# RemcoHoger/Space-Filling-Curves-for-Vision-Transformers

Measured on AMD Instinct MI355X. Metric: images/sec ViT-B/16 224px Hilbert-order training, higher is better.
Workload: dtype bf16; 1 GPU; vit_b16_224_hilbert: 224x224 Hilbert pixel order, 16x16-pixel tokens, batch 256/GPU, full train step (fwd+CE+bwd+clip+AdamW); global_batch=256, parallelism=dp1, hip_graph=False

## Files before the change

### space-filling-curves-for-vision-transformers_amd/csrc/gemm8p.hip

```cpp
#include "common_host.h"
#include "gemm_core.h"
#include <mutex>
#include <type_traits>
#include <unordered_map>

namespace sfcvit {
namespace {

using namespace gemm_core;

namespace p8 {

constexpr int T = 512, HALF = 16384, KTB = 65536, LDS_BYTES = 2 * KTB;
constexpr int LDS_TQ = LDS_BYTES, LDS_PATCH = LDS_TQ + 64, LDS_BIAS = LDS_PATCH + 8 * 2048, LDS_MAX = P8_LDS_MAX;
static_assert(LDS_BIAS == P8_LDS_BIAS, "dispatch.h prices the bias vector at this offset");
enum { RELU = P8_RELU, DROP = P8_DROP, RES = P8_RES, DACT = P8_DACT, CSUM = P8_CSUM, BITS = P8_BITS };

typedef const __attribute__((address_space(1))) void *gptr_t;
typedef __attribute__((address_space(3))) void *lptr_t;

template <int N> __device__ __forceinline__ void wait_vm() { asm volatile("s_waitcnt vmcnt(%0)" ::"n"(N) : "memory"); }
template <int N> __device__ __forceinline__ void wait_lgkm() {
    asm volatile("s_waitcnt lgkmcnt(%0)" ::"n"(N) : "memory");
    __builtin_amdgcn_sched_barrier(0);
// ... 16 lines not shown
};

template <int MASK>
__device__ __forceinline__ void epilogue_math(const sfcvit_gemm_args &g, int m, int n, float (&v)[16], const float (&bv)[16],
                                              const u32x4 (&side)[2], uint32_t thresh, float keep_scale, float dact_scale,
                                              uint32_t rk_in0, uint32_t rk_in1, u32x4 &w0, u32x4 &w1) {
    if (!(MASK & DACT)) {
#pragma unroll
        for (int r = 0; r < 16; r++) v[r] += bv[r];
    }
    if (MASK & RELU) {
#pragma unroll
        for (int r = 0; r < 16; r++) v[r] = fmaxf(v[r], 0.f);
    }
    if (MASK & DROP) {
        const uint64_t row = uint64_t(m) + uint64_t(uint32_t(g.row_offset));
        const uint32_t rk = mix32(uint32_t(row) * 0x9E3779B1u + ((row >> 32) ? rk_in1 : rk_in0));
#pragma unroll
        for (int p = 0; p < 8; p++) {
            bool k0, k1;
            drop_keep2(rk, uint32_t(n >> 1) + p, thresh, k0, k1);
            v[2 * p] = k0 ? v[2 * p] * keep_scale : 0.f;
            v[2 * p + 1] = k1 ? v[2 * p + 1] * keep_scale : 0.f;
        }
    }
    if (MASK & RES) {
        float rv[16];
        unpack8f(side[0], rv);
        unpack8f(side[1], rv + 8);
#pragma unroll
        for (int r = 0; r < 16; r++) v[r] += rv[r];
    }
    if ((MASK & BITS) && (MASK & RELU)) {
        uint32_t bits = 0;
#pragma unroll
        for (int r = 0; r < 16; r++) bits |= uint32_t(v[r] > 0.f) << r;
        uint8_t *mp = static_cast<uint8_t *>(g.actmask) + size_t(m) * g.ld_actmask + (n >> 3);
        asm volatile("global_store_short %0, %1, off\n\ts_nop 1" ::"v"(mp), "v"(bits) : "memory");
    }
    if (MASK & DACT) {
        if (MASK & BITS) {
            const uint32_t bits = side[0][0];
#pragma unroll
            for (int r = 0; r < 16; r++) v[r] = (bits >> r & 1u) ? v[r] * dact_scale : 0.f;
        } else {
            float a[16];
            unpack8f(side[0], a);
            unpack8f(side[1], a + 8);
#pragma unroll
            for (int r = 0; r < 16; r++) v[r] = a[r] > 0.f ? v[r] * dact_scale : 0.f;
        }
    }
    w0 = u32x4{pack2bf(v[0], v[1]), pack2bf(v[2], v[3]), pack2bf(v[4], v[5]), pack2bf(v[6], v[7])};
    w1 = u32x4{pack2bf(v[8], v[9]), pack2bf(v[10], v[11]), pack2bf(v[12], v[13]), pack2bf(v[14], v[15])};
}

#define SFCVIT_XROW(a, b) "ds_write_b128 %[wa], " a "\n\tds_write_b128 %[wb], " b "\n\tds_read_b128 " a ", %[ra]\n\tds_read_b128 " b ", %[ra] offset:1024\n\t"
template <int NR>
__device__ __forceinline__ void patch_exchange(u32x4 (&w)[NR][2], const StoreMap &sm) {
    static_assert(NR >= 1 && NR <= 8, "rows per batch");
    const int wa = sm.wa, wb = sm.wa ^ 16, ra = sm.ra;
    if constexpr (NR == 8)
        asm volatile(SFCVIT_XROW("%0", "%1") SFCVIT_XROW("%2", "%3") SFCVIT_XROW("%4", "%5") SFCVIT_XROW("%6", "%7")
                     SFCVIT_XROW("%8", "%9") SFCVIT_XROW("%10", "%11") SFCVIT_XROW("%12", "%13") SFCVIT_XROW("%14", "%15") "s_waitcnt lgkmcnt(0)"
                     : "+v"(w[0][0]), "+v"(w[0][1]), "+v"(w[1][0]), "+v"(w[1][1]), "+v"(w[2][0]), "+v"(w[2][1]), "+v"(w[3][0]), "+v"(w[3][1]),
                       "+v"(w[4][0]), "+v"(w[4][1]), "+v"(w[5][0]), "+v"(w[5][1]), "+v"(w[6][0]), "+v"(w[6][1]), "+v"(w[7][0]), "+v"(w[7][1])
                     : [wa] "v"(wa), [wb] "v"(wb), [ra] "v"(ra) : "memory");
    else if constexpr (NR == 7)
        asm volatile(SFCVIT_XROW("%0", "%1") SFCVIT_XROW("%2", "%3") SFCVIT_XROW("%4", "%5") SFCVIT_XROW("%6", "%7")
                     SFCVIT_XROW("%8", "%9") SFCVIT_XROW("%10", "%11") SFCVIT_XROW("%12", "%13") "s_waitcnt lgkmcnt(0)"
                     : "+v"(w[0][0]), "+v"(w[0][1]), "+v"(w[1][0]), "+v"(w[1][1]), "+v"(w[2][0]), "+v"(w[2][1]), "+v"(w[3][0]), "+v"(w[3][1]),
                       "+v"(w[4][0]), "+v"(w[4][1]), "+v"(w[5][0]), "+v"(w[5][1]), "+v"(w[6][0]), "+v"(w[6][1])
                     : [wa] "v"(wa), [wb] "v"(wb), [ra] "v"(ra) : "memory");
    else if constexpr (NR == 6)
        asm volatile(SFCVIT_XROW("%0", "%1") SFCVIT_XROW("%2", "%3") SFCVIT_XROW("%4", "%5") SFCVIT_XROW("%6", "%7")
                     SFCVIT_XROW("%8", "%9") SFCVIT_XROW("%10", "%11") "s_waitcnt lgkmcnt(0)"
                     : "+v"(w[0][0]), "+v"(w[0][1]), "+v"(w[1][0]), "+v"(w[1][1]), "+v"(w[2][0]), "+v"(w[2][1]), "+v"(w[3][0]), "+v"(w[3][1]),
                       "+v"(w[4][0]), "+v"(w[4][1]), "+v"(w[5][0]), "+v"(w[5][1])
                     : [wa] "v"(wa), [wb] "v"(wb), [ra] "v"(ra) : "memory");
    else if constexpr (NR == 4)
        asm volatile(SFCVIT_XROW("%0", "%1") SFCVIT_XROW("%2", "%3") SFCVIT_XROW("%4", "%5") SFCVIT_XROW("%6", "%7") "s_waitcnt lgkmcnt(0)"
                     : "+v"(w[0][0]), "+v"(w[0][1]), "+v"(w[1][0]), "+v"(w[1][1]), "+v"(w[2][0]), "+v"(w[2][1]), "+v"(w[3][0]), "+v"(w[3][1])
                     : [wa] "v"(wa), [wb] "v"(wb), [ra] "v"(ra) : "memory");
    else
        static_assert(NR == 8, "patch_exchange: batch sizes 4, 6, 7, 8");
}
#undef SFCVIT_XROW

__device__ __forceinline__ void store_row_pair(const sfcvit_gemm_args &g, int m, int n, const StoreMap &sm, const u32x4 &w0, const u32x4 &w1) {
    uint16_t *c = static_cast<uint16_t *>(g.c) + size_t(m) * g.ldc + n + sm.coff;
    asm volatile("global_store_dwordx4 %0, %1, off sc0 sc1 nt\n\ts_nop 1" ::"v"(c), "v"(w0) : "memory");
    asm volatile("global_store_dwordx4 %0, %1, off sc0 sc1 nt\n\ts_nop 1" ::"v"(c + size_t(8) * g.ldc), "v"(w1) : "memory");
}


template <int NI, int MASK, bool P2 = false>
__global__ __launch_bounds__(T) void gemm8p_kernel(const sfcvit_gemm_args g, unsigned *__restrict__ counters, int stag_slots, int stag_ticks, int walk) {
    constexpr int BM = 32 * NI, GR = 16 * NI;
    extern __shared__ __attribute__((aligned(16))) char smem[];
    if (stag_ticks > 0) {
        const uint64_t until = __builtin_amdgcn_s_memrealtime() + uint64_t((blockIdx.x >> 3) % stag_slots) * uint64_t(stag_ticks);
        while (__builtin_amdgcn_s_memrealtime() < until) __builtin_amdgcn_s_sleep(8);
    }
    const int tid = threadIdx.x, lane = tid & 63, wid = __builtin_amdgcn_readfirstlane(tid >> 6), wr = wid >> 2, wc = wid & 3;
    const int q = lane >> 4, nl = lane & 15;
    const int K = g.K, NT = g.N / 256, ntiles = ((g.M + BM - 1) / BM) * NT, KT = K / 64, m_last = g.M - BM;
    const uint16_t *A = static_cast<const uint16_t *>(g.a);
    const uint16_t *B = static_cast<const uint16_t *>(g.b);
    const int G = gridDim.x, per_xcd = G >> 3, xcd = blockIdx.x & 7;
    int *const tq = reinterpret_cast<int *>(smem + LDS_TQ);
    auto tile_of = [&](unsigned l) __attribute__((always_inline)) {
        const long t = long(l / unsigned(per_xcd)) * G + xcd * per_xcd + int(l % unsigned(per_xcd));
        if (t >= ntiles) return -1;
        if (walk > 0 && walk < NT) {
            const unsigned MT = unsigned(ntiles / NT), full = unsigned(NT / walk) * MT * unsigned(walk), ut = unsigned(t);
            const unsigned wcur = ut < full ? unsigned(walk) : unsigned(NT % walk), base = ut < full ? (ut / (MT * walk)) * walk : unsigned(NT / walk) * walk;
            const unsigned tt = ut < full ? ut % (MT * walk) : ut - full;
            return int((tt / wcur) << 16 | (base + tt % wcur));
        }
        return int((unsigned(t) / unsigned(NT)) << 16 | (unsigned(t) % unsigned(NT)));
    };
    auto finish = [&]() __attribute__((always_inline)) {
        if (tid == 0) {
            const unsigned old = atomicAdd(counters + 8, 1u);
            if (old == unsigned(G) - 1u) {
#pragma unroll
                for (int i = 0; i < 9; i++) counters[i] = 0u;
            }
        }
    };
    if (tid == 0) {
        const unsigned l0 = atomicAdd(counters + xcd, 1u);
        tq[0] = tile_of(l0);
        const unsigned l1 = atomicAdd(counters + xcd, 1u);
        tq[1] = tile_of(l1);
    }
    const bool has_bias = !(MASK & DACT) && g.bias != nullptr;
    if (has_bias)
        for (int i = tid; i < g.N / 8; i += T)
            *reinterpret_cast<u32x4 *>(smem + LDS_BIAS + i * 16) = static_cast<const u32x4 *>(g.bias)[i];
    __syncthreads();

    int tile_cur = __builtin_amdgcn_readfirstlane(tq[0]);
    if (tile_cur < 0) { finish(); return; }
    unsigned drawn = 0;
    if (tid == 0) drawn = atomicAdd(counters + xcd, 1u);
    const int tile_first = tile_cur;
    int t = 0;

    const int r1 = 8 * wid + (lane >> 3);
    const int sc = (lane & 7) ^ ((r1 >> 1) & 7);
    const int w1 = (r1 < GR - 64) ? r1 : r1 - (NI == 7 ? 16 : 32);
    const int b_row = (r1 >> 5) * 64 + ((r1 & 15) >> 2) * 16 + ((r1 >> 4) & 1) * 4 + (r1 & 3);
    const uint32_t voffA0 = (uint32_t(r1) * uint32_t(g.lda) + sc * 8) * 2, voffA1 = (uint32_t(64 + w1) * uint32_t(g.lda) + sc * 8) * 2;
    const uint32_t voffB = (uint32_t(b_row) * uint32_t(g.ldb) + sc * 8) * 2;
    const size_t a_second = size_t(GR) * g.lda, b_second = size_t(128) * g.ldb, b_h1 = size_t(8) * g.ldb;

    auto cursor_at = [&](int seq, int tile, bool is_a) __attribute__((always_inline)) {
        Cursor c;
        c.tile = seq;
        c.k0 = 0;
        if (tile < 0) tile = tile_first;
        c.p = is_a ? A + size_t(min((tile >> 16) * BM, m_last)) * g.lda : B + size_t(tile & 0xFFFF) * 256 * g.ldb;
        return c;
    };
    const uint16_t *next_a = nullptr, *next_b = nullptr;
    auto set_next = [&](int seq) __attribute__((always_inline)) {
        const Cursor na = cursor_at(seq, __builtin_amdgcn_readfirstlane(tq[seq & 3]), true);
        const Cursor nb = cursor_at(seq, __builtin_amdgcn_readfirstlane(tq[seq & 3]), false);
        next_a = na.p;
        next_b = nb.p;
    };
    auto advance = [&](Cursor &c, bool is_a) __attribute__((always_inline)) {
        if (c.k0 + 64 == K) { c.tile++; c.k0 = 0; c.p = is_a ? next_a : next_b; }
        else { c.k0 += 64; c.p += 64; }
    };
    const int m0_wave = wid * 1024;
    auto dma16 = [&](const uint16_t *base, uint32_t voff, int lds) __attribute__((always_inline)) {
        asm volatile("s_mov_b32 m0, %2\n\ts_nop 0\n\tglobal_load_lds_dwordx4 %0, %1"
                     :
                     : "v"(voff), "s"(base), "s"(lds)
                     : "memory");
    };
    auto stage_a = [&](const Cursor &c, int buf, int h) __attribute__((always_inline)) {
        const int d = m0_wave + buf * KTB + h * HALF;
        const uint32_t vo = h ? voffA1 : voffA0;
        dma16(c.p, vo, d);
        dma16(c.p + a_second, vo, d + 8192);
    };
    auto stage_b = [&](const Cursor &c, int buf, int h) __attribute__((always_inline)) {
        const uint16_t *p = c.p + (h ? b_h1 : 0);
        const int d = m0_wave + buf * KTB + 2 * HALF + h * HALF;
        dma16(p, voffB, d);
        dma16(p + b_second, voffB, d + 8192);
    };

    const int o0 = nl * 128 + ((q ^ ((nl >> 1) & 7)) << 4);
    const int a_off0 = wr * 8192 + o0, a_off1 = wr * 8192 + (o0 ^ 64);
    const int b_off0 = 2 * HALF + wc * 4096 + o0, b_off1 = 2 * HALF + wc * 4096 + (o0 ^ 64);
    bf16x8 fa0[4][2], fa1[NI - 4][2], fb0[2][2], fb1[2][2];
    auto read_a0 = [&](int buf) __attribute__((always_inline)) {
#pragma unroll
        for (int i = 0; i < 4; i++) {
            fa0[i][0] = *reinterpret_cast<const bf16x8 *>(smem + a_off0 + buf * KTB + i * 2048);
            fa0[i][1] = *reinterpret_cast<const bf16x8 *>(smem + a_off1 + buf * KTB + i * 2048);
        }
    };
    auto read_a1 = [&](int buf) __attribute__((always_inline)) {
#pragma unroll
        for (int i = 0; i < NI - 4; i++) {
            fa1[i][0] = *reinterpret_cast<const bf16x8 *>(smem + a_off0 + buf * KTB + HALF + i * 2048);
            fa1[i][1] = *reinterpret_cast<const bf16x8 *>(smem + a_off1 + buf * KTB + HALF + i * 2048);
        }
    };
    auto read_b = [&](bf16x8 (&fb)[2][2], int buf, int sub) __attribute__((always_inline)) {
#pragma unroll
        for (int j = 0; j < 2; j++) {
            fb[j][0] = *reinterpret_cast<const bf16x8 *>(smem + b_off0 + buf * KTB + sub * HALF + j * 2048);
            fb[j][1] = *reinterpret_cast<const bf16x8 *>(smem + b_off1 + buf * KTB + sub * HALF + j * 2048);
        }
    };

    f32x4 acc[NI][4];
    auto zero_acc = [&]() __attribute__((always_inline)) {
#pragma unroll
        for (int i = 0; i < NI; i++)
#pragma unroll
            for (int j = 0; j < 4; j++) acc[i][j] = f32x4{0.f, 0.f, 0.f, 0.f};
    };
    auto mma0 = [&](const bf16x8 (&fb)[2][2], int bsub) __attribute__((always_inline)) {
        __builtin_amdgcn_s_setprio(1);
#pragma unroll
        for (int kk = 0; kk < 2; kk++)
#pragma unroll
            for (int i = 0; i < 4; i++)
#pragma unroll
                for (int j = 0; j < 2; j++)
                    acc[i][bsub * 2 + j] = __builtin_amdgcn_mfma_f32_16x16x32_bf16(fb[j][kk], fa0[i][kk], acc[i][bsub * 2 + j], 0, 0, 0);
        __builtin_amdgcn_s_setprio(0);
    };
    auto mma1 = [&](const bf16x8 (&fb)[2][2], int bsub) __attribute__((always_inline)) {
        __builtin_amdgcn_s_setprio(1);
#pragma unroll
        for (int kk = 0; kk < 2; kk++)
#pragma unroll
            for (int i = 0; i < NI - 4; i++)
#pragma unroll
                for (int j = 0; j < 2; j++)
                    acc[4 + i][bsub * 2 + j] = __builtin_amdgcn_mfma_f32_16x16x32_bf16(fb[j][kk], fa1[i][kk], acc[4 + i][bsub * 2 + j], 0, 0, 0);
        __builtin_amdgcn_s_setprio(0);
    };

    const uint32_t thresh = (MASK & DROP) ? drop_thresh(g.dropout_p) : 0u;
    const float keep_scale = (MASK & DROP) ? 1.f / (1.f - g.dropout_p) : 1.f;
    const uint32_t seed_e = (MASK & DROP) ? eff_seed(g.dropout_seed, g.seed_off) : 0u;
    const uint32_t rk_in0 = (MASK & DROP) ? mix32(seed_e) : 0u, rk_in1 = (MASK & DROP) ? mix32(seed_e ^ 0x7FEB352Du) : 0u;
    const float dact_scale = g.dact_scale != 0.f ? g.dact_scale : 1.f;
    auto draw = [&]() __attribute__((always_inline)) {
        if (tid == 0) {
            tq[(t + 2) & 3] = tile_of(drawn);
            drawn = atomicAdd(counters + xcd, 1u);
        }
    };
    auto epilogue = [&]() __attribute__((always_inline)) {
        const int tile = tile_cur;
        int te = tid;
        asm volatile("" : "+v"(te));
        const int le = te & 63, qe = le >> 4, ne = le & 15;
        StoreMap sm;
        {
            const int patch = LDS_PATCH + wid * 2048, r0 = le >> 3, ch = le & 7;
            sm.wa = patch + ne * 128 + (((2 * qe) ^ (ne & 7)) << 4);
            sm.ra = patch + r0 * 128 + ((ch ^ r0) << 4);
            sm.coff = long(r0 - ne) * g.ldc + (8 * ch - 16 * qe);
        }
        const int m_new = (tile >> 16) * BM;
        const int m0 = min(m_new, m_last) + wr * GR + ne, n0 = (tile & 0xFFFF) * 256 + wc * 64 + qe * 16;
        mfma_fence();
        float bv[16];
        if (has_bias) {
            const char *bp = smem + LDS_BIAS + n0 * 2;
            unpack8f(*reinterpret_cast<const u32x4 *>(bp), bv);
            unpack8f(*reinterpret_cast<const u32x4 *>(bp + 16), bv + 8);
        } else {
#pragma unroll
            for (int r = 0; r < 16; r++) bv[r] = 0.f;
        }
        const uint16_t *sp = (MASK & RES) ? static_cast<const uint16_t *>(g.residual) : static_cast<const uint16_t *>(g.aux_in);
        const size_t ld_side = (MASK & RES) ? size_t(g.ldr) : size_t(g.ldaux);
        float cs[16];
#pragma unroll
        for (int r = 0; r < 16; r++) cs[r] = 0.f;
        auto batch = [&](auto i0c, auto i1c) __attribute__((always_inline)) {
            constexpr int i0 = decltype(i0c)::value, i1 = decltype(i1c)::value;
            u32x4 side[i1 - i0][2];
            if ((MASK & DACT) && (MASK & BITS)) {
#pragma unroll
                for (int i = i0; i < i1; i++)
                    side[i - i0][0][0] = *reinterpret_cast<const uint16_t *>(static_cast<const uint8_t *>(g.actmask) +
                                                                             size_t(m0 + 16 * i) * g.ld_actmask + (n0 >> 3));
            } else if (MASK & (RES | DACT)) {
#pragma unroll
                for (int i = i0; i < i1; i++) {
                    const uint16_t *p = sp + size_t(m0 + 16 * i) * ld_side + n0;
                    side[i - i0][0] = *reinterpret_cast<const u32x4 *>(p);
                    side[i - i0][1] = *reinterpret_cast<const u32x4 *>(p + 8);
                }
            }
            u32x4 pk[i1 - i0][2];
            static_for<i0, i1>([&](auto ic) __attribute__((always_inline)) {
                constexpr int i = decltype(ic)::value;
                float v[16] = {acc[i][0][0], acc[i][0][1], acc[i][0][2], acc[i][0][3], acc[i][1][0], acc[i][1][1],
                               acc[i][1][2], acc[i][1][3], acc[i][2][0], acc[i][2][1], acc[i][2][2], acc[i][2][3],
                               acc[i][3][0], acc[i][3][1], acc[i][3][2], acc[i][3][3]};
                epilogue_math<MASK>(g, m0 + 16 * i, n0, v, bv, side[i - i0], thresh, keep_scale, dact_scale, rk_in0, rk_in1,
                                    pk[i - i0][0], pk[i - i0][1]);
                if (MASK & CSUM) {
                    const bool own = m0 + 16 * i >= m_new;
#pragma unroll
                    for (int r = 0; r < 16; r++) cs[r] += own ? v[r] : 0.f;
                }
            });
            patch_exchange<i1 - i0>(pk, sm);
            static_for<i0, i1>([&](auto ic) __attribute__((always_inline)) {
                constexpr int i = decltype(ic)::value;
                store_row_pair(g, m0 + 16 * i, n0, sm, pk[i - i0][0], pk[i - i0][1]);
            });
        };
        if constexpr (NI == 8 && ((MASK & (DROP | RES)) == (DROP | RES) || (MASK & (DACT | CSUM | BITS)) == (DACT | CSUM))) {
            batch(std::integral_constant<int, 0>{}, std::integral_constant<int, 4>{});
            batch(std::integral_constant<int, 4>{}, std::integral_constant<int, NI>{});
        } else {
            batch(std::integral_constant<int, 0>{}, std::integral_constant<int, NI>{});
        }
        if (MASK & CSUM) {
#pragma unroll
            for (int r = 0; r < 16; r++) cs[r] = row16_sum(cs[r]);
            if (ne == 0) {
                float *pp = static_cast<float *>(g.workspace) + size_t(2 * (tile >> 16) + wr) * g.N + n0;
#pragma unroll
                for (int r4 = 0; r4 < 4; r4++)
                    *reinterpret_cast<f32x4 *>(pp + 4 * r4) = f32x4{cs[4 * r4], cs[4 * r4 + 1], cs[4 * r4 + 2], cs[4 * r4 + 3]};
            }
        }
        zero_acc();
    };

    Cursor ca = cursor_at(0, tile_cur, true), cb = cursor_at(0, tile_cur, false);
    stage_b(cb, 0, 0); stage_a(ca, 0, 0); stage_a(ca, 0, 1); stage_b(cb, 0, 1);
    advance(ca, true);
    advance(cb, false);
    if (P2) {
        stage_b(cb, 1, 0); stage_a(ca, 1, 0); stage_b(cb, 1, 1);
        advance(cb, false);
        wait_vm<6>();
    } else {
        stage_b(cb, 1, 0); stage_a(ca, 1, 0); stage_a(ca, 1, 1); stage_b(cb, 1, 1);
        advance(ca, true);
        advance(cb, false);
        wait_vm<8>();
    }
    bar();
    if (wr == 1) bar();
    zero_acc();

    constexpr int NSTORE = 2 * NI + ((MASK & CSUM) ? 4 : 0) + (((MASK & BITS) && (MASK & RELU)) ? NI : 0);
    auto stage_next = [&](int buf) __attribute__((always_inline)) {
        stage_a(ca, buf, 1);
        advance(ca, true);
        stage_b(cb, buf, 1);
        advance(cb, false);
        __builtin_amdgcn_sched_barrier(0);
    };
    auto ktile = [&](int buf, bool first, bool last) __attribute__((always_inline)) {
        read_b(fb0, buf, 0);
        read_a0(buf);
        bar();
        wait_lgkm<0>();
        mma0(fb0, 0);
        bar();
        read_a1(buf);
        bar();
        wait_lgkm<0>();
        mma1(fb0, 0);
        if (first) set_next(t + 1);
        bar();
        read_b(fb1, buf, 1);
        stage_b(cb, buf, 0);
        bar();
        wait_lgkm<0>();
        mma1(fb1, 1);
        bar();
        stage_a(ca, buf, 0);
        if (first && t > 0) wait_vm<4 + NSTORE>();
        else wait_vm<4>();
        bar();
        mma0(fb1, 1);
        if (last) {
            if (wr == 0) {
                bar();
                draw();
            }
            stage_next(buf);
            epilogue();
            if (wr == 1) bar();
        } else {
            bar();
            stage_next(buf);
        }
    };
    auto ktile2 = [&](int buf, bool first, bool last) __attribute__((always_inline)) {
        read_b(fb0, buf, 0);
        read_b(fb1, buf, 1);
        read_a0(buf);
        stage_a(ca, buf ^ 1, 1);
        advance(ca, true);
        __builtin_amdgcn_sched_barrier(0);
        if (first && t > 0) wait_vm<8 + NSTORE>();
        else wait_vm<8>();
        wait_lgkm<0>();
        bar();
        mma0(fb0, 0);
        mma0(fb1, 1);
        if (first) set_next(t + 1);
        bar();
        read_a1(buf);
        stage_b(cb, buf, 0);
        stage_a(ca, buf, 0);
        stage_b(cb, buf, 1);
        advance(cb, false);
        __builtin_amdgcn_sched_barrier(0);
        if (first && t > 0) wait_vm<8 + NSTORE>();
        else wait_vm<8>();
        wait_lgkm<0>();
        bar();
        mma1(fb0, 0);
        mma1(fb1, 1);
        if (last) {
            if (wr == 0) {
                bar();
                draw();
            }
            epilogue();
            if (wr == 1) bar();
// ... 309 lines not shown
```

### space-filling-curves-for-vision-transformers_amd/csrc/attention_bwd_fused.hip

```cpp
#include "attention_common.h"
#include "common_host.h"

namespace sfcvit {
namespace {

using namespace attn;

constexpr int FT = 1024, FWAVES = 16, FMAXC = 7;
static_assert(FUSED_MAX_N == 32 * FMAXC, "dispatch.h");

#ifdef SFCVIT_ISA_MARKERS
#define ISA_MARK(name) asm volatile("; ISA_MARK " name ::: "memory")
#else
#define ISA_MARK(name) do { } while (0)
#endif

#ifdef SFCVIT_ATTN_TRACE
__device__ unsigned long long g_attn_trace[512];
#define ATRACE(i) do { if (blockIdx.x == 5 && threadIdx.x == 0 && (i) < 512) g_attn_trace[(i)] = __builtin_amdgcn_s_memtime(); } while (0)
#else
#define ATRACE(i) do {} while (0)
#endif

__device__ __forceinline__ bf16x8 ds_tr_frag(const char *slot, int key0, int lane_off) {
    const char *pa = slot + key0 * 64 + lane_off;
    bf16x4 lo = __builtin_amdgcn_ds_read_tr16_b64_v4i16((SFCVIT_LDS bf16x4 *)pa);
    bf16x4 hi = __builtin_amdgcn_ds_read_tr16_b64_v4i16((SFCVIT_LDS bf16x4 *)(pa + 16 * 64));
    bf16x8 r;
    r[0] = lo[0]; r[1] = lo[1]; r[2] = lo[2]; r[3] = lo[3];
    r[4] = hi[0]; r[5] = hi[1]; r[6] = hi[2]; r[7] = hi[3];
    return r;
}

template <int NFC, bool DROP>
__global__ __launch_bounds__(FT) void attn_seq_bwd_fused_kernel(const sfcvit_attn_args a, int npad, int stag_round, int stag_per, int stag_ticks, int dq_sums, int items, int nt, unsigned *__restrict__ qcnt) {

    extern __shared__ __attribute__((aligned(16))) char smem[];
    stagger_start(stag_round, stag_per, stag_ticks);
    char *qimg = smem, *doimg = smem + npad * 128, *kimg0 = smem + 2 * npad * 128, *dsb = smem + 4 * npad * 128;
    char *small0 = dsb + 2 * npad * 64;
    unsigned long long *rec0 = reinterpret_cast<unsigned long long *>(smem + npad * FUSED_ROW_BYTES + 256);
    float *qpart = reinterpret_cast<float *>(smem + npad * FUSED_ROW_BYTES + 256 + 64);
    char *own_scratch = smem + npad * FUSED_ROW_BYTES + FUSED_EXTRA;
    const int tid = threadIdx.x, lane = tid & 63, wave = __builtin_amdgcn_readfirstlane(tid >> 6);
    const int N = a.N, D = a.H * HD, ld = 3 * D;
    const int nf = NFC ? NFC : (N + 15) >> 4, nc = NFC ? ((NFC + 1) >> 1) : npad >> 5;
    const bool split = nf <= FWAVES - 3;
    const int kfi = (split && wave == nf) ? nf - 1 : wave;
    const int tsel = !split ? -1 : wave == nf - 1 ? 0 : wave == nf ? 1 : -1;
    const bool is_key = wave < nf || (split && wave == nf), is_dq = wave >= FWAVES - 2;
    const uint32_t dth = drop_thresh(a.dropout_p);
    const float scale = a.scale, c2 = a.scale * LOG2E;
    const float dsc = 1.f / (1.f - a.dropout_p);
    const int g = lane >> 4, li = lane & 15;
    const int key = 16 * kfi + li;
    const uint32_t dth32 = dth << 16;

    bf16x8 vf[2];
    u32x4 opiece[2];
    auto fetch_item = [&](int it, char *small) __attribute__((always_inline)) {
        const int b = it / a.H, h = it - b * a.H;
        const uint16_t *vp = static_cast<const uint16_t *>(a.qkv) + size_t(b) * N * ld + h * HD + 2 * D;
#pragma unroll
        for (int kk = 0; kk < 2; kk++) vf[kk] = global_frag(vp, ld, 16 * kfi, is_key ? N : 0, kk, lane);
#pragma unroll
        for (int i = 0; i < 2; i++) {
            const int p = tid + FT * i, row = p >> 3, c = (p & 7) ^ kc_swz(row);
            opiece[i] = u32x4{0u, 0u, 0u, 0u};
            if (row < N) {
                const u32x4 *op = reinterpret_cast<const u32x4 *>(static_cast<const uint16_t *>(a.out) + (size_t(b) * N + row) * D + h * HD + c * 8);
                opiece[i] = nt ? __builtin_nontemporal_load(op) : *op;
            }
        }
        const float *lse = a.lse + bh_row(b, a.H, h, N, 0);
        float *lse_w = reinterpret_cast<float *>(small);
        uint32_t *rkey_w = reinterpret_cast<uint32_t *>(small) + 2 * npad;
        for (int i = tid; i < npad; i += FT) {
            lse_w[i] = lse_log2(lse, i, i < N, INFINITY);
            rkey_w[i] = mask_row_key(eff_seed(a.dropout_seed, a.seed_off), b, a.H, h, N, i);
        }
    };
    auto delta_item = [&](char *small) __attribute__((always_inline)) {
        float *del_w = reinterpret_cast<float *>(small) + npad;
#pragma unroll
        for (int i = 0; i < 2; i++) {
            const int p = tid + FT * i, row = p >> 3;
            float part = 0.f;
            if (p < npad * 8) {
                const u32x4 dpiece = *reinterpret_cast<const u32x4 *>(doimg + p * 16);
#pragma unroll
                for (int j = 0; j < 4; j++) {
                    part += __uint_as_float(dpiece[j] << 16) * __uint_as_float(opiece[i][j] << 16);
                    part += __uint_as_float(dpiece[j] & 0xFFFF0000u) * __uint_as_float(opiece[i][j] & 0xFFFF0000u);
                }
            }
            part += __shfl_xor(part, 1, 64);
            part += __shfl_xor(part, 2, 64);
            part += __shfl_xor(part, 4, 64);
            if ((tid & 7) == 0 && p < npad * 8) del_w[row] = part;
        }
    };
    const uint32_t lds_base = uint32_t(uintptr_t((lptr_t)smem));
    auto dma_piece = [&](const char *img, const uint16_t *src, int sld, int p) __attribute__((always_inline)) {
        const int row = p >> 3, cs = p & 7;
        const int c = cs ^ kc_swz(row);
        const uint16_t *gp = src + size_t(min(row, N - 1)) * sld + c * 8;
        const uint32_t m0v = __builtin_amdgcn_readfirstlane(lds_base + uint32_t(img - smem) + uint32_t(p) * 16u);
        if (nt) asm volatile("s_mov_b32 m0, %1\n\ts_nop 0\n\tglobal_load_lds_dwordx4 %0, off nt" ::"v"(gp), "s"(m0v) : "m0", "memory");
        else asm volatile("s_mov_b32 m0, %1\n\ts_nop 0\n\tglobal_load_lds_dwordx4 %0, off" ::"v"(gp), "s"(m0v) : "m0", "memory");
    };
    auto dma_wait = [&]() __attribute__((always_inline)) { asm volatile("s_waitcnt vmcnt(0)" ::: "memory"); };

    auto write_record = [&](int it, unsigned long long *rec) __attribute__((always_inline)) {
        const int b = it / a.H, h = it - b * a.H;
        rec[0] = reinterpret_cast<unsigned long long>(static_cast<const uint16_t *>(a.qkv) + size_t(b) * N * ld + h * HD);
        rec[1] = reinterpret_cast<unsigned long long>(static_cast<const uint16_t *>(a.dout) + size_t(b) * N * D + h * HD);
        rec[2] = reinterpret_cast<unsigned long long>(static_cast<uint16_t *>(a.dqkv) + size_t(b) * N * ld + h * HD);
    };
    int item = blockIdx.x, cur = 0;
    unsigned drawn = 0;
    if (qcnt && tid == 0) drawn = atomicAdd(qcnt, 1u);
    {
        const int b = item / a.H, h = item - b * a.H;
        const uint16_t *base = static_cast<const uint16_t *>(a.qkv) + size_t(b) * N * ld + h * HD;
        fetch_item(item, small0);
        if (tid == 0) write_record(item, rec0);
        dma_rows<FT, true>(qimg, base, ld, N, npad, tid, nt);
        dma_rows<FT, true>(doimg, static_cast<const uint16_t *>(a.dout) + size_t(b) * N * D + h * HD, D, N, npad, tid, nt);
        dma_rows<FT, true>(kimg0, base + D, ld, N, npad, tid, nt);
        {
            const int nz = (npad - 16 * nf) * 4;
            for (int i = tid; i < 2 * nz; i += FT) {
                char *dst = dsb + (i >= nz ? npad * 64 : 0) + 16 * nf * 64 + (i >= nz ? i - nz : i) * 16;
                *reinterpret_cast<u32x4 *>(dst) = u32x4{0u, 0u, 0u, 0u};
            }
        }
        __syncthreads();
        delta_item(small0);
        __syncthreads();
    }

  for (;;) {
    const int b = item / a.H, h = item - b * a.H;
    int nxt = items;
    bool has_next = false;
    char *kimg = kimg0 + cur * npad * 128, *knext = kimg0 + (cur ^ 1) * npad * 128;
    char *small = small0 + cur * 3 * npad * 4, *small_next = small0 + (cur ^ 1) * 3 * npad * 4;
    const float *lse_s = reinterpret_cast<const float *>(small), *del_s = lse_s + npad;
    const uint32_t *rkey_s = reinterpret_cast<const uint32_t *>(small) + 2 * npad;
    unsigned long long *rec = rec0 + cur * 4, *rec_next = rec0 + (cur ^ 1) * 4;
    if (tid == 0) {
        const int nx = qcnt ? int(gridDim.x + drawn) : item + int(gridDim.x);
        rec_next[3] = (unsigned long long)nx;
        if (nx < items) {
            write_record(nx, rec_next);
            if (qcnt) drawn = atomicAdd(qcnt, 1u);
        }
    }
    f32x4 dk[4], dv[4];
#pragma unroll
    for (int hf = 0; hf < 4; hf++) dk[hf] = dv[hf] = f32x4{0.f, 0.f, 0.f, 0.f};
    float ksum = 0.f;

    auto key_step = [&](int c) __attribute__((always_inline)) {
        int ln = lane;
        asm volatile("" : "+v"(ln));
        const int g = ln >> 4, li = ln & 15;
        const int k_off = lane_offsets(ln).k[0], t_off = lane_offsets(ln).t[0];
        const int key = 16 * kfi + li;
        const uint32_t key_g = uint32_t(key) * DROP_G;
        char *slot = dsb + (c & 1) * npad * 64;
        u32x2 pp[2], dd[2];
        const int ds_w = key * 64 + (((li >> 2) & 1) << 5) + 8 * g;
#pragma unroll
        for (int t = 0; t < 2; t++) {
            const int qf = 2 * c + t;
            if (tsel == 1 - t || 16 * qf >= N) {
                pp[t] = dd[t] = u32x2{0u, 0u};
                continue;
            }
            f32x4 s = {0.f, 0.f, 0.f, 0.f}, dp = {0.f, 0.f, 0.f, 0.f};
#pragma unroll
            for (int kk = 0; kk < 2; kk++) {
                s = __builtin_amdgcn_mfma_f32_16x16x32_bf16(kc_frag_at(qimg, 16 * qf, (k_off ^ (kk << 6))), kc_frag_at(kimg, 16 * kfi, (k_off ^ (kk << 6))), s, 0, 0, 0);
                dp = __builtin_amdgcn_mfma_f32_16x16x32_bf16(kc_frag_at(doimg, 16 * qf, (k_off ^ (kk << 6))), vf[kk], dp, 0, 0, 0);
            }
            const int ql0 = 16 * qf + 4 * g;
            const f32x4 lse4 = *reinterpret_cast<const f32x4 *>(lse_s + ql0);
            const f32x4 del4 = *reinterpret_cast<const f32x4 *>(del_s + ql0);
            const u32x4 rk4 = *reinterpret_cast<const u32x4 *>(rkey_s + ql0);
            float pr[4], dr[4];
#pragma unroll
            for (int r = 0; r < 4; r++) {
                const float pv = fast_exp2(s[r] * c2 - lse4[r]);
                float keep = 1.f;
                if (DROP)
                    keep = drop_hash_g(rk4[r], key_g) >= dth32 ? dsc : 0.f;
                pr[r] = pv * keep;
                dr[r] = pv * (dp[r] * keep - del4[r]);
            }
            if (16 * kfi + 16 > N) {
#pragma unroll
                for (int r = 0; r < 4; r++)
                    if (key >= N) dr[r] = 0.f;
            }
            ksum += (dr[0] + dr[1]) + (dr[2] + dr[3]);
            pp[t] = u32x2{pack2bf(pr[0], pr[1]), pack2bf(pr[2], pr[3])};
            dd[t] = u32x2{pack2bf(dr[0], dr[1]), pack2bf(dr[2], dr[3])};
        }
        const bf16x8 pf = __builtin_bit_cast(bf16x8, u32x4{pp[0][0], pp[0][1], pp[1][0], pp[1][1]});
        const bf16x8 dsf = __builtin_bit_cast(bf16x8, u32x4{dd[0][0], dd[0][1], dd[1][0], dd[1][1]});
        if (tsel != 1) *reinterpret_cast<u32x2 *>(slot + ds_w) = dd[0];
        if (tsel != 0) *reinterpret_cast<u32x2 *>(slot + (ds_w ^ 32)) = dd[1];
#pragma unroll
        for (int hf = 0; hf < 4; hf++) {
            dv[hf] = __builtin_amdgcn_mfma_f32_16x16x32_bf16(tr_frag_at(doimg, 32 * c, (t_off ^ (hf << 5))), pf, dv[hf], 0, 0, 0);
            dk[hf] = __builtin_amdgcn_mfma_f32_16x16x32_bf16(tr_frag_at(qimg, 32 * c, (t_off ^ (hf << 5))), dsf, dk[hf], 0, 0, 0);
        }
    };
    auto dq_step = [&](int c) __attribute__((always_inline)) {
        int ln = lane;
        asm volatile("" : "+v"(ln));
        const int g = ln >> 4, li = ln & 15;
        uint16_t *dq_base = reinterpret_cast<uint16_t *>(rec[2]);
        const char *slot = dsb + ((c - 1) & 1) * npad * 64;
        const int ds_r = (4 * g + (li >> 2)) * 64 + ((g & 1) << 5) + 8 * (li & 3);
        const int dqw = wave - (FWAVES - 2);
        int kt_off[2];
#pragma unroll
        for (int hh = 0; hh < 2; hh++) {
            const int col = 16 * (2 * dqw + hh) + 4 * (li & 3), tr = 4 * g + (li >> 2);
            kt_off[hh] = kc_off(tr, col >> 3) + ((col & 7) << 1);
        }
        f32x4 acc[2][2];
#pragma unroll
        for (int i = 0; i < 4; i++) acc[i >> 1][i & 1] = f32x4{0.f, 0.f, 0.f, 0.f};
        if (32 * (c - 1) + 16 < N) {
#pragma unroll
            for (int ks = 0; ks < FMAXC; ks++) {
                if (ks < nc) {
                    const bf16x8 b0 = ds_tr_frag(slot, 32 * ks, ds_r), b1 = ds_tr_frag(slot, 32 * ks, ds_r ^ 32);
#pragma unroll
                    for (int hh = 0; hh < 2; hh++) {
                        const bf16x8 kt = tr_frag_at(kimg, 32 * ks, kt_off[hh]);
                        acc[hh][0] = __builtin_amdgcn_mfma_f32_16x16x32_bf16(kt, b0, acc[hh][0], 0, 0, 0);
                        acc[hh][1] = __builtin_amdgcn_mfma_f32_16x16x32_bf16(kt, b1, acc[hh][1], 0, 0, 0);
                    }
                }
            }
        } else {
#pragma unroll
            for (int ks = 0; ks < FMAXC; ks++) {
                if (ks < nc) {
                    const bf16x8 b0 = ds_tr_frag(slot, 32 * ks, ds_r);
#pragma unroll
                    for (int hh = 0; hh < 2; hh++)
                        acc[hh][0] = __builtin_amdgcn_mfma_f32_16x16x32_bf16(tr_frag_at(kimg, 32 * ks, kt_off[hh]), b0, acc[hh][0], 0, 0, 0);
                }
            }
        }
        mfma_fence();
#pragma unroll
        for (int qf = 0; qf < 2; qf++) {
            const int q = 32 * (c - 1) + 16 * qf + li;
            const auto lo = __builtin_amdgcn_permlane16_swap(pack2bf(acc[0][qf][0] * scale, acc[0][qf][1] * scale),
                                                             pack2bf(acc[1][qf][0] * scale, acc[1][qf][1] * scale), false, false);
            const auto hi = __builtin_amdgcn_permlane16_swap(pack2bf(acc[0][qf][2] * scale, acc[0][qf][3] * scale),
                                                             pack2bf(acc[1][qf][2] * scale, acc[1][qf][3] * scale), false, false);
            const u32x4 o = {lo[0], hi[0], lo[1], hi[1]};
            if (q < N) *reinterpret_cast<u32x4 *>(dq_base + size_t(q) * ld + 32 * dqw + 16 * (g & 1) + 8 * (g >> 1)) = o;
        }
    };
    auto prefetch = [&](int c) __attribute__((always_inline)) {
        int te = tid;
        asm volatile("" : "+v"(te));
        const uint16_t *nq = reinterpret_cast<const uint16_t *>(rec_next[0]);
        if (c == 1) {
            if (te < FT - 128)
                for (int p = te; p < npad * 8; p += FT - 128) dma_piece(knext, nq + D, ld, p);
        }
        if (te < 512) {
            const int p = (c - 1) * 256 + (te & 255);
            if (te < 256) dma_piece(qimg, nq, ld, p);
            else dma_piece(doimg, reinterpret_cast<const uint16_t *>(rec_next[1]), D, p);
        }
    };
    [[maybe_unused]] int tr_i = ((item - int(blockIdx.x)) / int(gridDim.x)) * 16;
    ATRACE(tr_i);
    for (int c = 0; c < nc; c++) {
        if (has_next && c >= 1) prefetch(c);
        if (is_key) {
            ISA_MARK("key_step begin");
            key_step(c);
            ISA_MARK("key_step end");
        } else if (is_dq && c >= 1) {
            ISA_MARK("dq_step begin");
            dq_step(c);
            ISA_MARK("dq_step end");
        }
        if (!is_dq) dma_wait();
        __syncthreads();
        if (c == 0) {
            nxt = __builtin_amdgcn_readfirstlane(int(rec_next[3]));
            has_next = nxt < items;
        }
        ATRACE(tr_i + 1 + c);
    }
    if (has_next) prefetch(nc);
    if (is_dq) dq_step(nc);
    if (has_next) fetch_item(nxt, small_next);
    ATRACE(tr_i + 8);
    if (a.colsum_part && dq_sums && is_key) {
        int ln = lane;
        asm volatile("" : "+v"(ln));
        const int g = ln >> 4, li = ln & 15, key = 16 * kfi + li;
        float sk = ksum;
        {
            const auto h = __builtin_amdgcn_permlane32_swap(__float_as_uint(sk), __float_as_uint(sk), false, false);
            sk = __uint_as_float(h[0]) + __uint_as_float(h[1]);
            const auto q = __builtin_amdgcn_permlane16_swap(__float_as_uint(sk), __float_as_uint(sk), false, false);
            sk = __uint_as_float(q[0]) + __uint_as_float(q[1]);
        }
        if (key >= N) sk = 0.f;
#pragma unroll
        for (int hc = 0; hc < 2; hc++) {
            const u32x4 kv = *reinterpret_cast<const u32x4 *>(kimg + kc_off(key, 2 * g + hc));
#pragma unroll
            for (int e = 0; e < 4; e++) {
                const float q0 = row16_sum(sk * bf2f(uint16_t(kv[e]))), q1 = row16_sum(sk * bf2f(uint16_t(kv[e] >> 16)));
                if (li == 0) {
                    qpart[wave * 64 + 16 * g + 8 * hc + 2 * e] = q0 * scale;
                    qpart[wave * 64 + 16 * g + 8 * hc + 2 * e + 1] = q1 * scale;
                }
            }
        }
    }
    float *px = reinterpret_cast<float *>(own_scratch);
    if (split && wave == nf) {
        mfma_fence();
#pragma unroll
        for (int hf = 0; hf < 4; hf++)
#pragma unroll
            for (int r = 0; r < 4; r++) {
                px[(4 * hf + r) * 64 + lane] = dk[hf][r];
                px[(16 + 4 * hf + r) * 64 + lane] = dv[hf][r];
            }
    }
    asm volatile("s_waitcnt vmcnt(0)" : "+v"(vf[0]), "+v"(vf[1]), "+v"(opiece[0]), "+v"(opiece[1]) :: "memory");
    __syncthreads();
    ATRACE(tr_i + 9);
#ifdef SFCVIT_ATTN_TRACE
    if (blockIdx.x == 5 && (threadIdx.x & 63) == 0 && tr_i == 16) g_attn_trace[288 + (threadIdx.x >> 6)] = __builtin_amdgcn_s_memtime();
#endif
    if (split && wave == nf - 1) {
        mfma_fence();
#pragma unroll
        for (int hf = 0; hf < 4; hf++)
#pragma unroll
            for (int r = 0; r < 4; r++) {
                dk[hf][r] += px[(4 * hf + r) * 64 + lane];
                dv[hf][r] += px[(16 + 4 * hf + r) * 64 + lane];
            }
    }
    const bool owns = wave < nf;
    if (owns) {
        mfma_fence();
        uint16_t *dbase = reinterpret_cast<uint16_t *>(rec[2]);
        store_rows(dbase + D, ld, key, key < N, dk, scale, lane);
        store_rows(dbase + 2 * D, ld, key, key < N, dv, 1.f, lane);
    }
    if (a.colsum_part) {
        float *cs = reinterpret_cast<float *>(npad * 128 >= FUSED_CS_BYTES ? kimg : own_scratch + FUSED_POST_BYTES);
        if (owns) {
#pragma unroll
            for (int hf = 0; hf < 4; hf++)
#pragma unroll
                for (int r = 0; r < 4; r++) {
                    const float sk = row16_sum(key < N ? dk[hf][r] : 0.f), sv = row16_sum(key < N ? dv[hf][r] : 0.f);
                    if (li == 0) {
                        cs[wave * 128 + 16 * hf + 4 * g + r] = sk * scale;
                        cs[wave * 128 + 64 + 16 * hf + 4 * g + r] = sv;
                    }
                }
        }
        __syncthreads();
        if (tid < 192) {
            const int third = tid >> 6, c = tid & 63;
            float s = 0.f;
            if (third == 0) {
                if (dq_sums)
                    for (int w = 0; w < nf + (split ? 1 : 0); w++) s += qpart[w * 64 + c];
            } else {
                for (int w = 0; w < nf; w++) s += cs[w * 128 + (third - 1) * 64 + c];
            }
            if (third || dq_sums) a.colsum_part[size_t(b) * 3 * D + third * D + h * HD + c] = s;
        }
    }
    ATRACE(tr_i + 10);
    if (!has_next) break;
#ifdef SFCVIT_ATTN_TRACE
    if (blockIdx.x == 5 && (threadIdx.x & 63) == 0 && tr_i == 16) g_attn_trace[256 + (threadIdx.x >> 6)] = __builtin_amdgcn_s_memtime();
#endif
    __syncthreads();
    ATRACE(tr_i + 12);
    delta_item(small_next);
    ATRACE(tr_i + 13);
    __syncthreads();
    ATRACE(tr_i + 11);
    item = nxt;
    cur ^= 1;
  }
    if (qcnt && tid == 0) {
        const unsigned old = atomicAdd(qcnt + 1, 1u);
        if (old == gridDim.x - 1u) { qcnt[0] = 0u; qcnt[1] = 0u; }
    }
}

template <int NFC, bool DROP>
int launch(const AttnPlan &p, const sfcvit_attn_args &a, unsigned *qcnt, hipStream_t s) {
    if (int rc = raise_lds_limit(reinterpret_cast<const void *>(&attn_seq_bwd_fused_kernel<NFC, DROP>), FUSED_MAX_LDS, "attention_bwd_fused attribute")) return rc;
    hipLaunchKernelGGL((attn_seq_bwd_fused_kernel<NFC, DROP>), dim3(p.grid), dim3(FT), p.lds, s, a, p.npad, p.round, p.per, p.ticks, p.dq_sums,
                       a.B * a.H, p.nt, qcnt);
    return check_launch("attention_bwd_fused");
}

}

int attn_seq_bwd_fused(const AttnPlan &p, const sfcvit_attn_args &a, hipStream_t s) {
    unsigned *slot = p.queue ? stream_counters(s) : nullptr;
    unsigned *qcnt = slot ? slot + 12 : nullptr;
    if (p.inst == 13) return p.drop ? launch<13, true>(p, a, qcnt, s) : launch<13, false>(p, a, qcnt, s);
    return p.drop ? launch<0, true>(p, a, qcnt, s) : launch<0, false>(p, a, qcnt, s);
}

#ifdef SFCVIT_ATTN_TRACE
extern "C" int sfcvit_debug_attn_trace(unsigned long long *out) {
    return hipMemcpyFromSymbol(out, HIP_SYMBOL(g_attn_trace), sizeof(unsigned long long) * 512) == hipSuccess ? 0 : 1;
}
#endif
}
```

Measured before the change: 8184 images/s.

## Overlap persistent GEMM prologue: static first tile, async tile draws, deferred bias/seed loads

Each block now takes its first tile statically from blockIdx and issues its tile-queue atomics as asynchronous returning atomics. The bias vector and dropout seed are loaded into registers and only written to LDS after the first A/B stages are in flight, which removes the initial __syncthreads and the serialized atomic round-trips before the main loop. Tail handling for the end of the queue now points the next-tile cursors at the last K slice of the current tile. The dropout+residual epilogue is also split into smaller 2/2/4-row batches, and ReLU+dropout+bits gets a 4/4 split, to cut register pressure. The change depends on hand-tuned vmcnt counts and on the tile_of offset by per_xcd matching the static first tile, so a mistake there could break correctness.

```diff
diff --git a/space-filling-curves-for-vision-transformers_amd/csrc/gemm8p.hip b/space-filling-curves-for-vision-transformers_amd/csrc/gemm8p.hip
--- a/space-filling-curves-for-vision-transformers_amd/csrc/gemm8p.hip
+++ b/space-filling-curves-for-vision-transformers_amd/csrc/gemm8p.hip
@@ -122,8 +122,12 @@
         asm volatile(SFCVIT_XROW("%0", "%1") SFCVIT_XROW("%2", "%3") SFCVIT_XROW("%4", "%5") SFCVIT_XROW("%6", "%7") "s_waitcnt lgkmcnt(0)"
                      : "+v"(w[0][0]), "+v"(w[0][1]), "+v"(w[1][0]), "+v"(w[1][1]), "+v"(w[2][0]), "+v"(w[2][1]), "+v"(w[3][0]), "+v"(w[3][1])
                      : [wa] "v"(wa), [wb] "v"(wb), [ra] "v"(ra) : "memory");
+    else if constexpr (NR == 2)
+        asm volatile(SFCVIT_XROW("%0", "%1") SFCVIT_XROW("%2", "%3") "s_waitcnt lgkmcnt(0)"
+                     : "+v"(w[0][0]), "+v"(w[0][1]), "+v"(w[1][0]), "+v"(w[1][1])
+                     : [wa] "v"(wa), [wb] "v"(wb), [ra] "v"(ra) : "memory");
     else
-        static_assert(NR == 8, "patch_exchange: batch sizes 4, 6, 7, 8");
+        static_assert(NR == 8, "patch_exchange: batch sizes 2, 4, 6, 7, 8");
 }
 #undef SFCVIT_XROW
 
@@ -169,23 +173,32 @@
             }
         }
     };
+    int tile_cur = __builtin_amdgcn_readfirstlane(tile_of(unsigned(blockIdx.x) >> 3));
+    if (tile_cur < 0) { finish(); return; }
+    unsigned *const queue = counters + xcd;
+    auto draw_async = [&](unsigned &dst) __attribute__((always_inline)) {
+        asm volatile("s_nop 4\n\tglobal_atomic_add %0, %1, %2, %3 sc0" : "=&v"(dst) : "v"(0), "v"(1u), "s"(queue) : "memory");
+    };
+    unsigned drawn1 = 0, drawn = 0;
     if (tid == 0) {
-        const unsigned l0 = atomicAdd(counters + xcd, 1u);
-        tq[0] = tile_of(l0);
-        const unsigned l1 = atomicAdd(counters + xcd, 1u);
-        tq[1] = tile_of(l1);
+        draw_async(drawn1);
+        draw_async(drawn);
     }
     const bool has_bias = !(MASK & DACT) && g.bias != nullptr;
-    if (has_bias)
-        for (int i = tid; i < g.N / 8; i += T)
-            *reinterpret_cast<u32x4 *>(smem + LDS_BIAS + i * 16) = static_cast<const u32x4 *>(g.bias)[i];
-    __syncthreads();
-
-    int tile_cur = __builtin_amdgcn_readfirstlane(tq[0]);
-    if (tile_cur < 0) { finish(); return; }
-    unsigned drawn = 0;
-    if (tid == 0) drawn = atomicAdd(counters + xcd, 1u);
-    const int tile_first = tile_cur;
+    static_assert(BIAS_MAX_N <= 16 * T, "two bias pieces per thread");
+    const int nbias = has_bias ? g.N / 8 : 0;
+    u32x4 bias0, bias1;
+    if constexpr (!(MASK & DACT)) {
+        const u32x4 *bsrc = has_bias ? static_cast<const u32x4 *>(g.bias) : static_cast<const u32x4 *>(g.b);
+        const int last = has_bias ? nbias - 1 : 0;
+        asm volatile("global_load_dwordx4 %0, %1, off" : "=&v"(bias0) : "v"(bsrc + min(tid, last)) : "memory");
+        asm volatile("global_load_dwordx4 %0, %1, off" : "=&v"(bias1) : "v"(bsrc + min(tid + T, last)) : "memory");
+    }
+    uint32_t seed_word = 0u;
+    if constexpr (MASK & DROP) {
+        const uint32_t *wp = g.seed_off ? g.seed_off : static_cast<const uint32_t *>(g.b);
+        asm volatile("global_load_dword %0, %1, off" : "=&v"(seed_word) : "v"(wp) : "memory");
+    }
     int t = 0;
 
     const int r1 = 8 * wid + (lane >> 3);
@@ -200,16 +213,15 @@
         Cursor c;
         c.tile = seq;
         c.k0 = 0;
-        if (tile < 0) tile = tile_first;
         c.p = is_a ? A + size_t(min((tile >> 16) * BM, m_last)) * g.lda : B + size_t(tile & 0xFFFF) * 256 * g.ldb;
         return c;
     };
     const uint16_t *next_a = nullptr, *next_b = nullptr;
     auto set_next = [&](int seq) __attribute__((always_inline)) {
-        const Cursor na = cursor_at(seq, __builtin_amdgcn_readfirstlane(tq[seq & 3]), true);
-        const Cursor nb = cursor_at(seq, __builtin_amdgcn_readfirstlane(tq[seq & 3]), false);
-        next_a = na.p;
-        next_b = nb.p;
+        const int nxt = __builtin_amdgcn_readfirstlane(tq[seq & 3]);
+        const int tail = nxt < 0 ? K - 192 : 0;
+        next_a = cursor_at(seq, nxt < 0 ? tile_cur : nxt, true).p + tail;
+        next_b = cursor_at(seq, nxt < 0 ? tile_cur : nxt, false).p + tail;
     };
     auto advance = [&](Cursor &c, bool is_a) __attribute__((always_inline)) {
         if (c.k0 + 64 == K) { c.tile++; c.k0 = 0; c.p = is_a ? next_a : next_b; }
@@ -293,13 +305,13 @@
 
     const uint32_t thresh = (MASK & DROP) ? drop_thresh(g.dropout_p) : 0u;
     const float keep_scale = (MASK & DROP) ? 1.f / (1.f - g.dropout_p) : 1.f;
-    const uint32_t seed_e = (MASK & DROP) ? eff_seed(g.dropout_seed, g.seed_off) : 0u;
-    const uint32_t rk_in0 = (MASK & DROP) ? mix32(seed_e) : 0u, rk_in1 = (MASK & DROP) ? mix32(seed_e ^ 0x7FEB352Du) : 0u;
+    uint32_t rk_in0 = 0u, rk_in1 = 0u;
     const float dact_scale = g.dact_scale != 0.f ? g.dact_scale : 1.f;
     auto draw = [&]() __attribute__((always_inline)) {
         if (tid == 0) {
-            tq[(t + 2) & 3] = tile_of(drawn);
-            drawn = atomicAdd(counters + xcd, 1u);
+            asm volatile("" : "+v"(drawn));
+            tq[(t + 2) & 3] = tile_of(drawn + unsigned(per_xcd));
+            draw_async(drawn);
         }
     };
     auto epilogue = [&]() __attribute__((always_inline)) {
@@ -367,7 +379,12 @@
                 store_row_pair(g, m0 + 16 * i, n0, sm, pk[i - i0][0], pk[i - i0][1]);
             });
         };
-        if constexpr (NI == 8 && ((MASK & (DROP | RES)) == (DROP | RES) || (MASK & (DACT | CSUM | BITS)) == (DACT | CSUM))) {
+        if constexpr (NI == 8 && (MASK & (DROP | RES)) == (DROP | RES)) {
+            batch(std::integral_constant<int, 0>{}, std::integral_constant<int, 2>{});
+            batch(std::integral_constant<int, 2>{}, std::integral_constant<int, 4>{});
+            batch(std::integral_constant<int, 4>{}, std::integral_constant<int, 8>{});
+        } else if constexpr (NI == 8 && ((MASK & (DACT | CSUM | BITS)) == (DACT | CSUM) ||
+                                  (MASK & (RELU | DROP | BITS)) == (RELU | DROP | BITS))) {
             batch(std::integral_constant<int, 0>{}, std::integral_constant<int, 4>{});
             batch(std::integral_constant<int, 4>{}, std::integral_constant<int, NI>{});
         } else {
@@ -393,13 +410,29 @@
     if (P2) {
         stage_b(cb, 1, 0); stage_a(ca, 1, 0); stage_b(cb, 1, 1);
         advance(cb, false);
-        wait_vm<6>();
+        wait_vm<14>();
     } else {
         stage_b(cb, 1, 0); stage_a(ca, 1, 0); stage_a(ca, 1, 1); stage_b(cb, 1, 1);
         advance(ca, true);
         advance(cb, false);
-        wait_vm<8>();
-    }
+        wait_vm<16>();
+    }
+    asm volatile("" : "+v"(drawn1));
+    if constexpr (!(MASK & DACT)) {
+        asm volatile("" : "+v"(bias0), "+v"(bias1));
+        if (tid < nbias) *reinterpret_cast<u32x4 *>(smem + LDS_BIAS + tid * 16) = bias0;
+        if (tid + T < nbias) *reinterpret_cast<u32x4 *>(smem + LDS_BIAS + (tid + T) * 16) = bias1;
+    }
+    if constexpr (MASK & DROP) {
+        asm volatile("" : "+v"(seed_word));
+        const uint32_t seed_e = __builtin_amdgcn_readfirstlane(g.seed_off ? g.dropout_seed + seed_word : g.dropout_seed);
+        rk_in0 = mix32(seed_e);
+        rk_in1 = mix32(seed_e ^ 0x7FEB352Du);
+    }
+    if (tid == 0) tq[1] = tile_of(drawn1 + unsigned(per_xcd));
+    if (P2) wait_vm<6>();
+    else wait_vm<8>();
+    wait_lgkm<0>();
     bar();
     if (wr == 1) bar();
     zero_acc();
```

After: 8244 images/s, median of 6. Within noise of the previous version (+0.7%).

## Overlap attention-bwd epilogue: DMA-stage LSE, DPP column sums, earlier delta

Applied to the files above, without the earlier changes.

The next item's LSE values are loaded straight into LDS with global_load_lds during the prefetch phase, so fetch_item only rescales them instead of issuing its own global loads. The per-row16 column sums of dK/dV now use a DPP butterfly scatter, so each lane produces one value rather than running 32 full row reductions. delta_item for the next item moves ahead of the colsum barrier, which removes one __syncthreads per item, and waves 6 and up issue their dK/dV stores after the colsum work. The aim is a shorter serial epilogue per item, in exchange for more intricate lane-slot mapping and tighter LDS reuse ordering.

```diff
diff --git a/space-filling-curves-for-vision-transformers_amd/csrc/attention_bwd_fused.hip b/space-filling-curves-for-vision-transformers_amd/csrc/attention_bwd_fused.hip
--- a/space-filling-curves-for-vision-transformers_amd/csrc/attention_bwd_fused.hip
+++ b/space-filling-curves-for-vision-transformers_amd/csrc/attention_bwd_fused.hip
@@ -18,8 +18,10 @@
 #ifdef SFCVIT_ATTN_TRACE
 __device__ unsigned long long g_attn_trace[512];
 #define ATRACE(i) do { if (blockIdx.x == 5 && threadIdx.x == 0 && (i) < 512) g_attn_trace[(i)] = __builtin_amdgcn_s_memtime(); } while (0)
+#define ATRACEX(ti, j) do { if (blockIdx.x == 5 && threadIdx.x == 0 && (ti) < 256) g_attn_trace[320 + ((ti) >> 1) + (j)] = __builtin_amdgcn_s_memtime(); } while (0)
 #else
 #define ATRACE(i) do {} while (0)
+#define ATRACEX(ti, j) do {} while (0)
 #endif
 
 __device__ __forceinline__ bf16x8 ds_tr_frag(const char *slot, int key0, int lane_off) {
@@ -30,6 +32,30 @@
     r[0] = lo[0]; r[1] = lo[1]; r[2] = lo[2]; r[3] = lo[3];
     r[4] = hi[0]; r[5] = hi[1]; r[6] = hi[2]; r[7] = hi[3];
     return r;
+}
+
+template <int CTRL>
+__device__ __forceinline__ float dpp_f32(float v) {
+    return __builtin_bit_cast(float, __builtin_amdgcn_update_dpp(0, __builtin_bit_cast(int, v), CTRL, 0xF, 0xF, true));
+}
+template <int CTRL, int NV>
+__device__ __forceinline__ void row16_scatter_step(float (&x)[16], bool hi) {
+#pragma unroll
+    for (int m = 0; m < NV / 2; m++) {
+        const float keep = hi ? x[2 * m + 1] : x[2 * m], send = hi ? x[2 * m] : x[2 * m + 1];
+        x[m] = keep + dpp_f32<CTRL>(send);
+    }
+}
+__device__ __forceinline__ int row16_slot(int li) {
+    const int j = li & 3, q0 = (li >> 2) & 1, q1 = li >> 3;
+    return 8 * q1 + 4 * (q0 ^ q1) + (j ^ (3 * q0));
+}
+__device__ __forceinline__ void row16_scatter(float (&x)[16], int li) {
+    const int s = row16_slot(li);
+    row16_scatter_step<0xB1, 16>(x, s & 1);
+    row16_scatter_step<0x4E, 8>(x, (s >> 1) & 1);
+    row16_scatter_step<0x141, 4>(x, (s >> 2) & 1);
+    row16_scatter_step<0x140, 2>(x, (s >> 3) & 1);
 }
 
 template <int NFC, bool DROP>
@@ -45,6 +71,7 @@
     const int tid = threadIdx.x, lane = tid & 63, wave = __builtin_amdgcn_readfirstlane(tid >> 6);
     const int N = a.N, D = a.H * HD, ld = 3 * D;
     const int nf = NFC ? NFC : (N + 15) >> 4, nc = NFC ? ((NFC + 1) >> 1) : npad >> 5;
+    const bool lse_staged = nc >= 2;
     const bool split = nf <= FWAVES - 3;
     const int kfi = (split && wave == nf) ? nf - 1 : wave;
     const int tsel = !split ? -1 : wave == nf - 1 ? 0 : wave == nf ? 1 : -1;
@@ -52,13 +79,14 @@
     const uint32_t dth = drop_thresh(a.dropout_p);
     const float scale = a.scale, c2 = a.scale * LOG2E;
     const float dsc = 1.f / (1.f - a.dropout_p);
-    const int g = lane >> 4, li = lane & 15;
+    const int li = lane & 15;
     const int key = 16 * kfi + li;
     const uint32_t dth32 = dth << 16;
 
     bf16x8 vf[2];
     u32x4 opiece[2];
-    auto fetch_item = [&](int it, char *small) __attribute__((always_inline)) {
+    const uint32_t seed = eff_seed(a.dropout_seed, a.seed_off);
+    auto fetch_item = [&](int it, char *small, bool staged) __attribute__((always_inline)) {
         const int b = it / a.H, h = it - b * a.H;
         const uint16_t *vp = static_cast<const uint16_t *>(a.qkv) + size_t(b) * N * ld + h * HD + 2 * D;
 #pragma unroll
@@ -76,8 +104,8 @@
         float *lse_w = reinterpret_cast<float *>(small);
         uint32_t *rkey_w = reinterpret_cast<uint32_t *>(small) + 2 * npad;
         for (int i = tid; i < npad; i += FT) {
-            lse_w[i] = lse_log2(lse, i, i < N, INFINITY);
-            rkey_w[i] = mask_row_key(eff_seed(a.dropout_seed, a.seed_off), b, a.H, h, N, i);
+            lse_w[i] = staged ? (i < N ? lse_w[i] * LOG2E : INFINITY) : lse_log2(lse, i, i < N, INFINITY);
+            rkey_w[i] = mask_row_key(seed, b, a.H, h, N, i);
         }
     };
     auto delta_item = [&](char *small) __attribute__((always_inline)) {
@@ -109,6 +137,11 @@
         if (nt) asm volatile("s_mov_b32 m0, %1\n\ts_nop 0\n\tglobal_load_lds_dwordx4 %0, off nt" ::"v"(gp), "s"(m0v) : "m0", "memory");
         else asm volatile("s_mov_b32 m0, %1\n\ts_nop 0\n\tglobal_load_lds_dwordx4 %0, off" ::"v"(gp), "s"(m0v) : "m0", "memory");
     };
+    auto stage_lse = [&](int it, char *small, int te) __attribute__((always_inline)) {
+        const float *gp = a.lse + size_t(it) * N + min(te, N - 1);
+        const uint32_t m0v = __builtin_amdgcn_readfirstlane(lds_base + uint32_t(small - smem) + uint32_t(te) * 4u);
+        asm volatile("s_mov_b32 m0, %1\n\ts_nop 0\n\tglobal_load_lds_dword %0, off" ::"v"(gp), "s"(m0v) : "m0", "memory");
+    };
     auto dma_wait = [&]() __attribute__((always_inline)) { asm volatile("s_waitcnt vmcnt(0)" ::: "memory"); };
 
     auto write_record = [&](int it, unsigned long long *rec) __attribute__((always_inline)) {
@@ -123,7 +156,7 @@
     {
         const int b = item / a.H, h = item - b * a.H;
         const uint16_t *base = static_cast<const uint16_t *>(a.qkv) + size_t(b) * N * ld + h * HD;
-        fetch_item(item, small0);
+        fetch_item(item, small0, false);
         if (tid == 0) write_record(item, rec0);
         dma_rows<FT, true>(qimg, base, ld, N, npad, tid, nt);
         dma_rows<FT, true>(doimg, static_cast<const uint16_t *>(a.dout) + size_t(b) * N * D + h * HD, D, N, npad, tid, nt);
@@ -278,6 +311,7 @@
         if (c == 1) {
             if (te < FT - 128)
                 for (int p = te; p < npad * 8; p += FT - 128) dma_piece(knext, nq + D, ld, p);
+            if (lse_staged && te < npad) stage_lse(nxt, small_next, te);
         }
         if (te < 512) {
             const int p = (c - 1) * 256 + (te & 255);
@@ -308,7 +342,7 @@
     }
     if (has_next) prefetch(nc);
     if (is_dq) dq_step(nc);
-    if (has_next) fetch_item(nxt, small_next);
+    if (has_next) fetch_item(nxt, small_next, lse_staged);
     ATRACE(tr_i + 8);
     if (a.colsum_part && dq_sums && is_key) {
         int ln = lane;
@@ -335,6 +369,7 @@
             }
         }
     }
+    ATRACEX(tr_i, 0);
     float *px = reinterpret_cast<float *>(own_scratch);
     if (split && wave == nf) {
         mfma_fence();
@@ -346,6 +381,9 @@
                 px[(16 + 4 * hf + r) * 64 + lane] = dv[hf][r];
             }
     }
+#ifdef SFCVIT_ATTN_TRACE
+    if (blockIdx.x == 5 && (threadIdx.x & 63) == 0 && tr_i == 16) g_attn_trace[272 + (threadIdx.x >> 6)] = __builtin_amdgcn_s_memtime();
+#endif
     asm volatile("s_waitcnt vmcnt(0)" : "+v"(vf[0]), "+v"(vf[1]), "+v"(opiece[0]), "+v"(opiece[1]) :: "memory");
     __syncthreads();
     ATRACE(tr_i + 9);
@@ -363,27 +401,42 @@
             }
     }
     const bool owns = wave < nf;
-    if (owns) {
+    auto store_item = [&]() __attribute__((always_inline)) {
         mfma_fence();
         uint16_t *dbase = reinterpret_cast<uint16_t *>(rec[2]);
         store_rows(dbase + D, ld, key, key < N, dk, scale, lane);
         store_rows(dbase + 2 * D, ld, key, key < N, dv, 1.f, lane);
-    }
+    };
+    const bool stores_late = a.colsum_part && wave >= 6;
+    if (owns && !stores_late) store_item();
+    ATRACEX(tr_i, 1);
+    if (has_next) delta_item(small_next);
+    ATRACEX(tr_i, 4);
     if (a.colsum_part) {
         float *cs = reinterpret_cast<float *>(npad * 128 >= FUSED_CS_BYTES ? kimg : own_scratch + FUSED_POST_BYTES);
         if (owns) {
+            int ln = lane;
+            asm volatile("" : "+v"(ln));
+            const int g = ln >> 4, li = ln & 15;
+            float xk[16], xv[16];
 #pragma unroll
             for (int hf = 0; hf < 4; hf++)
 #pragma unroll
-                for (int r = 0; r < 4; r++) {
-                    const float sk = row16_sum(key < N ? dk[hf][r] : 0.f), sv = row16_sum(key < N ? dv[hf][r] : 0.f);
-                    if (li == 0) {
-                        cs[wave * 128 + 16 * hf + 4 * g + r] = sk * scale;
-                        cs[wave * 128 + 64 + 16 * hf + 4 * g + r] = sv;
-                    }
-                }
-        }
+                for (int r = 0; r < 4; r++) xk[4 * hf + r] = dk[hf][r], xv[4 * hf + r] = dv[hf][r];
+            if (16 * kfi + 16 > N) {
+#pragma unroll
+                for (int k = 0; k < 16; k++) xk[k] = 16 * kfi + li < N ? xk[k] : 0.f, xv[k] = 16 * kfi + li < N ? xv[k] : 0.f;
+            }
+            row16_scatter(xk, li);
+            row16_scatter(xv, li);
+            const int s = row16_slot(li), col = 16 * (s >> 2) + 4 * g + (s & 3);
+            cs[wave * 128 + col] = xk[0] * scale;
+            cs[wave * 128 + 64 + col] = xv[0];
+        }
+        if (owns && stores_late) store_item();
+        ATRACEX(tr_i, 2);
         __syncthreads();
+        ATRACEX(tr_i, 3);
         if (tid < 192) {
             const int third = tid >> 6, c = tid & 63;
             float s = 0.f;
@@ -402,10 +455,6 @@
     if (blockIdx.x == 5 && (threadIdx.x & 63) == 0 && tr_i == 16) g_attn_trace[256 + (threadIdx.x >> 6)] = __builtin_amdgcn_s_memtime();
 #endif
     __syncthreads();
-    ATRACE(tr_i + 12);
-    delta_item(small_next);
-    ATRACE(tr_i + 13);
-    __syncthreads();
     ATRACE(tr_i + 11);
     item = nxt;
     cur ^= 1;
```

Measured after the change: 8093 images/s before, 8119 images/s after, median of 6. No clear change (+0.3%).
